# epruesse/SINA

Hardware: AMD Instinct MI355X
Metric: aligned sequences/sec (whole node), 100k full-length 16S vs SILVA-NR-scale ref (higher is better)
Workload: dtype f32

## Files before the change

sina_amd/csrc/graph_build.hip:

```cpp
#include <algorithm>
#include <cstring>
#include <type_traits>

#include "common.h"
#include "ctx.h"

namespace sina_hip {
namespace {

#ifndef SINA_GRAPH_THREADS
#define SINA_GRAPH_THREADS 512
#endif
#ifndef SINA_GRAPH_MINWAVES
#define SINA_GRAPH_MINWAVES 8
#endif
constexpr int kGT = SINA_GRAPH_THREADS;
constexpr uint32_t kNoPrev = 0xFFFFu;
constexpr int kMaxFam = kFamilyMax;
#ifndef SINA_GRAPH_KTC
#define SINA_GRAPH_KTC 128
#endif
#ifndef SINA_GRAPH_TNW
#define SINA_GRAPH_TNW 512
#endif
constexpr int kTC = SINA_GRAPH_KTC;
constexpr int kTNW = SINA_GRAPH_TNW;
static_assert(kTC % 64 == 0 && kTC < 255 && kTNW >= 32 && kTNW % 2 == 0, "tile geometry");
static_assert((kMaxFam * (kTC / 64) + SINA_GRAPH_THREADS / 64 - 1) / (SINA_GRAPH_THREADS / 64) <= 64, "far-entry flags of a wave fit 64 bits");

#ifdef SINA_DP_PROFILE
__device__ unsigned long long g_graph_prof[16];
#define GP_DECL unsigned long long gp_[16] = {}; unsigned long long gt_ = __builtin_amdgcn_s_memtime();
#define GP(i) { const unsigned long long t_ = __builtin_amdgcn_s_memtime(); gp_[i] += t_ - gt_; gt_ = t_; }
#define GP_FLUSH if (threadIdx.x == 0) { for (int i_ = 0; i_ < 16; i_++) atomicAdd(&g_graph_prof[i_], gp_[i_]); }
#else
#define GP_DECL
#define GP(i)
#define GP_FLUSH
#endif

struct GraphArgs {
    const uint32_t *ref_ab;
    const uint64_t *ref_off;
    const uint32_t *fam_ids;
    const uint64_t *fam_off;
    const uint64_t *pred_off;
    const float *wtab;
    uint4 *rec;
    uint32_t *node_pos;
    uint32_t *succ_min;
    uint32_t *far_mark;
    uint32_t *pred;
    uint2 *pred4;
    uint32_t *sizes;
    uint16_t *chain_rows;
    uint32_t width, ncap;
    uint32_t tile_bytes;
    uint32_t bitmap_off;
    uint32_t member_off;
    uint32_t member_cap;
    uint32_t fam_cap;
    int W;
    int want_smin;
    uint2 *reach;
    float kappa64;
};

struct Member {
    uint64_t beg;
    uint32_t len;
    uint32_t cur, curn;
    uint32_t carry, carryn;
    uint32_t id;
};
static_assert(sizeof(Member) == 32, "LDS layout");
constexpr uint32_t kOCpos = 0;
constexpr uint32_t kONbase = kOCpos + 4 * kTC;
constexpr uint32_t kOPres = kONbase + 4 * (kTC + 2);
constexpr uint32_t kOWA = kOPres + 4 * kTC;
constexpr uint32_t kOWC = kOWA + 4 * kTNW;
constexpr uint32_t kOWD = kOWC + 4 * kTNW;
constexpr uint32_t kOWB = (kOWD + 4 * kTNW + 7) & ~7u;
constexpr uint32_t kOLi = kOWB + 8 * kTNW;
constexpr uint32_t kONn = kOLi + 32 * kTC;
constexpr uint32_t kONfar = kONn + kTC;
constexpr uint32_t kOMask = kONfar + kTNW;
constexpr uint32_t kONcol = kOMask + kTNW;
constexpr uint32_t kOE = (kONcol + kTNW + 15) & ~15u;
constexpr int kELower0Bit = 14;
constexpr uint32_t kODot16 = kTC + 1;

template <typename In, typename Out>
__device__ uint32_t block_exscan(const In *in, Out *out, uint32_t n, uint32_t *tmp) {
    const uint32_t tid = threadIdx.x;
    const uint32_t chunk = (n + kGT - 1) / kGT;
    const uint32_t b = min(n, tid * chunk), e = min(n, b + chunk);
    uint32_t s = 0;
    for (uint32_t i = b; i < e; i++) s += (uint32_t)in[i];
    uint32_t x = s;
    const int lane = tid & 63, wave = tid >> 6;
#pragma unroll
    for (int off = 1; off < 64; off <<= 1) {
        const uint32_t y = __shfl_up(x, off);
        if (lane >= off) x += y;
    }
    if (lane == 63) tmp[wave] = x;
    __syncthreads();
    uint32_t base = 0, total = 0;
    for (int w = 0; w < kGT / 64; w++) {
        if (w < wave) base += tmp[w];
        total += tmp[w];
    }
    uint32_t run = base + x - s;
    __syncthreads();
    for (uint32_t i = b; i < e; i++) {
        const uint32_t v = (uint32_t)in[i];
        out[i] = (Out)run;
        run += v;
    }
    __syncthreads();
    return total;
}

template <typename Get, typename Out>
__device__ uint32_t block_exscan_f(uint32_t n, Get get, Out *out, uint32_t *tmp) {
    const uint32_t tid = threadIdx.x;
    const uint32_t chunk = (n + kGT - 1) / kGT;
    const uint32_t b = min(n, tid * chunk), e = min(n, b + chunk);
    uint32_t s = 0;
    for (uint32_t i = b; i < e; i++) s += get(i);
    uint32_t x = s;
    const int lane = tid & 63, wave = tid >> 6;
#pragma unroll
    for (int off = 1; off < 64; off <<= 1) {
        const uint32_t y = __shfl_up(x, off);
        if (lane >= off) x += y;
    }
    if (lane == 63) tmp[wave] = x;
    __syncthreads();
    uint32_t base = 0, total = 0;
    for (int w = 0; w < kGT / 64; w++) {
        if (w < wave) base += tmp[w];
        total += tmp[w];
    }
    uint32_t run = base + x - s;
    __syncthreads();
    for (uint32_t i = b; i < e; i++) {
        const uint32_t v = get(i);
        out[i] = (Out)run;
        run += v;
    }
    __syncthreads();
    return total;
}

__device__ __attribute__((noinline)) void fill_tile(const uint32_t *__restrict__ ref_ab, uint32_t bitmap_off, uint32_t member_off,
                                                    uint32_t nwords, uint32_t n_tasks, uint32_t c0, uint32_t tc) {
    extern __shared__ __attribute__((aligned(16))) unsigned char smem[];
    uint32_t *cposT = reinterpret_cast<uint32_t *>(smem + kOCpos);
    uint32_t *presT = reinterpret_cast<uint32_t *>(smem + kOPres);
    uint16_t *eE = reinterpret_cast<uint16_t *>(smem + kOE);
    const uint32_t *bitmap = reinterpret_cast<const uint32_t *>(smem + bitmap_off);
    const uint16_t *wrank = reinterpret_cast<const uint16_t *>(bitmap + nwords);
    Member *mb = reinterpret_cast<Member *>(smem + member_off);
    constexpr uint32_t kEAbsent = 0x00FFu, kEFirst = 1u << 13;
    constexpr uint32_t kCH = kTC / 64, kNW = kGT / 64;
    const uint32_t wave = (uint32_t)__builtin_amdgcn_readfirstlane((int)(threadIdx.x >> 6));
    const uint32_t lane = threadIdx.x & 63u;
    auto rank = [&](uint32_t pos) -> uint32_t {
        return (uint32_t)wrank[pos >> 5] + __popc(bitmap[pos >> 5] & ((1u << (pos & 31)) - 1u));
    };
        for (uint32_t t4 = wave; t4 < n_tasks; t4 += 8 * kNW) {
            uint32_t abv[8];
#pragma unroll
            for (int u = 0; u < 8; u++) {
                const uint32_t task = t4 + (uint32_t)u * kNW;
                abv[u] = 0xFFFFFFFFu;
                if (task < n_tasks) {
                    const uint32_t j = task / kCH;
                    const uint32_t cur = (uint32_t)__builtin_amdgcn_readfirstlane((int)mb[j].cur);
                    const uint32_t len = (uint32_t)__builtin_amdgcn_readfirstlane((int)mb[j].len);
                    const uint64_t beg = mb[j].beg;
                    const uint64_t begs = ((uint64_t)(uint32_t)__builtin_amdgcn_readfirstlane((int)(uint32_t)(beg >> 32)) << 32) |
                                          (uint32_t)__builtin_amdgcn_readfirstlane((int)(uint32_t)beg);
                    const uint32_t i = cur + (task % kCH) * 64u + lane;
                    if (i < len) abv[u] = ref_ab[begs + i];
                }
            }
#pragma unroll
            for (int u = 0; u < 8; u++) {
                const uint32_t task = t4 + (uint32_t)u * kNW;
                if (task >= n_tasks) continue;
                const uint32_t j = task / kCH, slot0 = (task % kCH) * 64u, slot = slot0 + lane;
                const uint32_t cur = (uint32_t)__builtin_amdgcn_readfirstlane((int)mb[j].cur);
                uint32_t ev = kEAbsent;
                if (abv[u] != 0xFFFFFFFFu) {
                    const uint32_t ab = abv[u];
                    const uint32_t pos = ab & 0xFFFFFFu;
                    const uint32_t c = rank(pos) - c0;
                    if (c < tc) {
                        const uint32_t m = (ab >> 24) & 0x1Fu;
                        ev = c | (m << 8) | (cur + slot == 0 ? kEFirst : 0u);
                        atomicOr(&presT[c], 1u << m);
                        cposT[c] = pos;
                    }
                }
                eE[j * (uint32_t)kTC + slot] = (uint16_t)ev;
                const uint32_t n_in = (uint32_t)__popcll(__builtin_amdgcn_ballot_w64(ev != kEAbsent));
                if (n_in && lane == 0) atomicMax(&mb[j].curn, cur + slot0 + n_in);
            }
        }
}

__device__ __forceinline__ uint32_t node_of_entry(uint32_t ev) {
    extern __shared__ __attribute__((aligned(16))) unsigned char smem[];
    const uint32_t *nbaseT = reinterpret_cast<const uint32_t *>(smem + kONbase);
    const uint32_t *presT = reinterpret_cast<const uint32_t *>(smem + kOPres);
    const uint8_t *liOf = smem + kOLi;
    const uint32_t c = ev & 0xFFu, m = (ev >> 8) & 31u;
    const uint32_t b = nbaseT[c];
    return b + liOf[b + __popc(presT[c] & ((1u << m) - 1u))];
}
__device__ __attribute__((noinline)) void merge_dot16(uint32_t n_tasks) {
    extern __shared__ __attribute__((aligned(16))) unsigned char smem[];
    const uint32_t *presT = reinterpret_cast<const uint32_t *>(smem + kOPres);
    uint16_t *eE = reinterpret_cast<uint16_t *>(smem + kOE);
    for (uint32_t e = threadIdx.x; e < n_tasks * 64u; e += kGT) {
        const uint32_t ev = eE[e];
        const uint32_t c = ev & 0xFFu;
        if (c != 0xFFu && ((ev >> 8) & 31u) == 16u && !(presT[c] & 0x10000u)) eE[e] = (uint16_t)((ev & ~(31u << 8)) | (1u << kELower0Bit));
    }
}
__device__ __attribute__((noinline)) void fix_dot16(uint32_t n_tasks, uint32_t ca, uint32_t cb, uint32_t w0) {
    extern __shared__ __attribute__((aligned(16))) unsigned char smem[];
    const uint32_t *nbaseT = reinterpret_cast<const uint32_t *>(smem + kONbase);
    const uint32_t *wC = reinterpret_cast<const uint32_t *>(smem + kOWC);
    const uint16_t *eE = reinterpret_cast<const uint16_t *>(smem + kOE);
    uint8_t *maskN = smem + kOMask;
    for (uint32_t e = threadIdx.x; e < n_tasks * 64u; e += kGT) {
        const uint32_t ev = eE[e];
        const uint32_t c = ev & 0xFFu;
        if (c >= ca && c < cb && (ev >> kELower0Bit) && wC[nbaseT[c] - w0] == e / (uint32_t)kTC) maskN[node_of_entry(ev) - w0] = 16;
    }
}
__global__ void __launch_bounds__(kGT) __attribute__((amdgpu_waves_per_eu(SINA_GRAPH_MINWAVES, SINA_GRAPH_MINWAVES))) family_graph_kernel(GraphArgs a) {
    extern __shared__ __attribute__((aligned(16))) unsigned char smem[];
    __shared__ uint32_t s_tmp[kGT / 64 + 8];
    const uint32_t q = blockIdx.x, tid = threadIdx.x;
    const uint32_t nwords = (a.width + 31) / 32;
    const uint64_t f0 = a.fam_off[q];
    const uint32_t F = (uint32_t)(a.fam_off[q + 1] - f0);
    uint32_t *cposT = reinterpret_cast<uint32_t *>(smem + kOCpos);
    uint32_t *nbaseT = reinterpret_cast<uint32_t *>(smem + kONbase);
    uint32_t *presT = reinterpret_cast<uint32_t *>(smem + kOPres);
    uint32_t *wA = reinterpret_cast<uint32_t *>(smem + kOWA);
    uint32_t *wC = reinterpret_cast<uint32_t *>(smem + kOWC);
    uint32_t *wD = reinterpret_cast<uint32_t *>(smem + kOWD);
    unsigned long long *wB = reinterpret_cast<unsigned long long *>(smem + kOWB);
    uint8_t *liOf = smem + kOLi;
    uint8_t *nn = smem + kONn;
    uint8_t *nfarN = smem + kONfar;
    uint8_t *maskN = smem + kOMask;
    uint8_t *ncolN = smem + kONcol;
    uint16_t *eE = reinterpret_cast<uint16_t *>(smem + kOE);
    uint32_t *bitmap = reinterpret_cast<uint32_t *>(smem + a.bitmap_off);
    uint16_t *wrank = reinterpret_cast<uint16_t *>(bitmap + nwords);
    Member *mb = reinterpret_cast<Member *>(smem + a.member_off);
    constexpr uint32_t kEFirst = 1u << 13;
    constexpr uint32_t kCH = kTC / 64, kNW = kGT / 64;
    const uint32_t wave = (uint32_t)__builtin_amdgcn_readfirstlane((int)(threadIdx.x >> 6));
    const uint32_t lane = threadIdx.x & 63u;
    const uint32_t n_tasks = F * kCH;

    uint32_t *sz = a.sizes + kBuiltWords * (size_t)q;
    for (uint32_t j = tid; j < F; j += kGT) {
        const uint32_t id = a.fam_ids[f0 + j];
        mb[j].id = id;
        mb[j].beg = a.ref_off[id];
        mb[j].len = (uint32_t)(a.ref_off[id + 1] - a.ref_off[id]);
        mb[j].cur = mb[j].curn = 0;
        mb[j].carry = mb[j].carryn = kNoPrev;
    }
    for (uint32_t i = tid; i < nwords; i += kGT) bitmap[i] = 0;
    if (tid == 0) nbaseT[kODot16] = 0;
    __syncthreads();
    GP_DECL

    for (uint32_t j0 = 0; j0 < F; j0 += 8) {
        uint32_t maxlen = 0;
#pragma unroll
        for (int u = 0; u < 8; u++) maxlen = max(maxlen, j0 + u < F ? mb[j0 + u].len : 0u);
        for (uint32_t i = tid; i < maxlen; i += kGT) {
            uint32_t ab[8];
#pragma unroll
            for (int u = 0; u < 8; u++)
                ab[u] = (j0 + u < F && i < mb[j0 + u].len) ? a.ref_ab[mb[j0 + u].beg + i] : 0xFFFFFFFFu;
#pragma unroll
            for (int u = 0; u < 8; u++)
                if (ab[u] != 0xFFFFFFFFu) {
                    const uint32_t pos = ab[u] & 0xFFFFFFu;
                    atomicOr(&bitmap[pos >> 5], 1u << (pos & 31));
                }
        }
    }
    __syncthreads();
    GP(0)
    {
        const uint32_t chunk = (nwords + kGT - 1) / kGT;
        const uint32_t b = min(nwords, tid * chunk), e = min(nwords, b + chunk);
        uint32_t s = 0;
        for (uint32_t i = b; i < e; i++) s += __popc(bitmap[i]);
        uint32_t x = s;
        const int lane = tid & 63, wave = tid >> 6;
#pragma unroll
        for (int off = 1; off < 64; off <<= 1) {
            const uint32_t y = __shfl_up(x, off);
            if (lane >= off) x += y;
        }
        if (lane == 63) s_tmp[wave] = x;
        __syncthreads();
        uint32_t base = 0, total = 0;
        for (int w = 0; w < kGT / 64; w++) {
            if (w < wave) base += s_tmp[w];
            total += s_tmp[w];
        }
        uint32_t run = base + x - s;
        for (uint32_t i = b; i < e; i++) {
            wrank[i] = (uint16_t)run;
            run += __popc(bitmap[i]);
        }
        if (tid == 0) s_tmp[kGT / 64] = total;
    }
    __syncthreads();
    const uint32_t NC = s_tmp[kGT / 64];
    if (NC > 65535u) {
        if (tid == 0) {
            sz[kBuiltN] = NC;
            sz[kBuiltEdges] = sz[kBuiltSpill] = 0;
            sz[kBuiltStatus] = kBuiltNodeCap;
        }
        return;
    }
    auto rank = [&](uint32_t pos) -> uint32_t {
        return (uint32_t)wrank[pos >> 5] + __popc(bitmap[pos >> 5] & ((1u << (pos & 31)) - 1u));
    };
    uint4 *rec = a.rec + (size_t)q * a.ncap;
    uint32_t *node_pos = a.node_pos + (size_t)q * a.ncap;
    uint32_t *smin = a.succ_min + (size_t)q * a.ncap;
    uint32_t *last = a.far_mark + (size_t)q * a.ncap;
    uint32_t *pred = a.pred + a.pred_off[q];
    uint16_t *chain_rows = a.chain_rows + (size_t)q * a.ncap;
    const float *wt = a.wtab + (size_t)F * (kMaxFam + 1);
    uint32_t N = 0, E = 0;
    GP(1)

    for (uint32_t c0 = 0; c0 < NC; c0 += kTC) {
        const uint32_t tc = min((uint32_t)kTC, NC - c0);
        for (uint32_t i = tid; i < (uint32_t)kTC; i += kGT) presT[i] = 0;
        __syncthreads();
        GP(2)
        fill_tile(a.ref_ab, a.bitmap_off, a.member_off, nwords, n_tasks, c0, tc);
        __syncthreads();
        for (uint32_t c = tid; c < tc; c += kGT) {
            uint32_t p = presT[c];
            if ((p & 0x10001u) == 0x10001u) {
                p &= ~0x10000u;
                presT[c] = p;
                nbaseT[kODot16] = 1u;
            }
            nn[c] = (uint8_t)__popc(p);
        }
        __syncthreads();
        if (nbaseT[kODot16]) {
            merge_dot16(n_tasks);
            __syncthreads();
        }
        GP(3)
        const uint32_t tn = block_exscan(nn, nbaseT, tc, s_tmp);
        if (tid == 0) nbaseT[tc] = tn;
        for (uint32_t ln = tid; ln < tn; ln += kGT)
            if (N + ln < a.ncap) {
                last[N + ln] = 0;
                if (a.want_smin) smin[N + ln] = 0xFFFFFFFFu;
            }
        __syncthreads();
        GP(5)
        uint32_t te = 0;
        for (uint32_t ca = 0; ca < tc;) {
            const uint32_t w0 = nbaseT[ca];
            uint32_t cb = tc;
            if (tn - w0 > (uint32_t)kTNW) {
                uint32_t lo = ca + 1, hi = tc;
                while (lo < hi) {
                    const uint32_t mid = (lo + hi + 1) / 2;
                    if (nbaseT[mid] - w0 <= (uint32_t)kTNW) lo = mid;
                    else hi = mid - 1;
                }
                cb = lo;
            }
            const uint32_t wn = nbaseT[cb] - w0;
            for (uint32_t i = tid; i < wn; i += kGT) {
                wA[i] = 0;
                wB[i] = 0;
                wC[i] = 0xFFFFFFFFu;
                nfarN[i] = 0;
            }
            __syncthreads();
            for (uint32_t task = wave; task < n_tasks; task += kNW) {
                const uint32_t j = task / kCH, slot = (task % kCH) * 64u + lane;
                const uint32_t ev = eE[j * (uint32_t)kTC + slot];
                const uint32_t c = ev & 0xFFu;
                if (c >= ca && c < cb) {
                    const uint32_t m = (ev >> 8) & 31u;
                    atomicMin(&wC[nbaseT[c] + __popc(presT[c] & ((1u << m) - 1u)) - w0], j);
                }
            }
            __syncthreads();
            for (uint32_t c = ca + tid; c < cb; c += kGT) {
                const uint32_t base = nbaseT[c], k = nn[c];
                uint32_t pp = presT[c];
                for (uint32_t x = 0; x < k; x++) {
                    const uint32_t mj = wC[base - w0 + x];
                    uint32_t r = 0;
                    for (uint32_t y = 0; y < k; y++) r += (wC[base - w0 + y] < mj) ? 1u : 0u;
                    liOf[base + x] = (uint8_t)r;
                    maskN[base - w0 + r] = (uint8_t)(__ffs(pp) - 1);
                    ncolN[base - w0 + r] = (uint8_t)c;
                    pp &= pp - 1u;
                }
            }
            __syncthreads();
            if (nbaseT[kODot16]) {
                fix_dot16(n_tasks, ca, cb, w0);
                __syncthreads();
            }
            GP(4)
            auto node_of = [&](uint32_t ev) -> uint32_t { return node_of_entry(ev); };
            unsigned long long farbits = 0;
            {
                uint32_t it = 0;
                for (uint32_t task = wave; task < n_tasks; task += kNW, it++) {
                    const uint32_t j = task / kCH, slot = (task % kCH) * 64u + lane;
                    const uint32_t ev = eE[j * (uint32_t)kTC + slot];
                    const uint32_t c = ev & 0xFFu;
                    const bool mine = c >= ca && c < cb;
                    const uint32_t ln = mine ? node_of(ev) : 0u;
                    uint32_t lnp = __shfl_up(ln, 1);
                    const bool left_mine = __shfl_up(mine ? 1 : 0, 1) != 0;
                    if (!mine) continue;
                    const uint32_t node = N + ln;
                    const bool first = (ev & kEFirst) != 0;
                    atomicAdd(&wA[ln - w0], first ? 1u : 0x10001u);
                    if (mb[j].cur + slot + 1 == mb[j].curn) mb[j].carryn = node;
                    if (j == 0 && mb[0].cur + slot < a.ncap) chain_rows[mb[0].cur + slot] = (uint16_t)node;
                    if (!first) {
                        if (slot && (lane == 0 || !left_mine)) lnp = node_of(eE[j * (uint32_t)kTC + slot - 1]);
                        const uint32_t pn = slot ? N + lnp : mb[j].carry;
                        const uint32_t d = node - pn;
                        if (d <= 64u) atomicOr(&wB[ln - w0], 1ull << (d - 1u));
                        else farbits |= 1ull << it;
                    }
                }
            }
            for (uint32_t i = tid; i < wn; i += kGT) wC[i] = 0xFFFFFFFFu;
            __syncthreads();
            GP(6)
            const uint32_t te_w = block_exscan_f(wn, [&](uint32_t i) { return wA[i] >> 16; }, wD, s_tmp);
            while (__syncthreads_or(farbits != 0 ? 1 : 0)) {
                uint32_t it = 0;
                for (uint32_t task = wave; task < n_tasks; task += kNW, it++) {
                    if (!((farbits >> it) & 1ull)) continue;
                    const uint32_t j = task / kCH, slot = (task % kCH) * 64u + lane;
                    const uint32_t ln = node_of(eE[j * (uint32_t)kTC + slot]);
                    const uint32_t pn = slot ? N + node_of(eE[j * (uint32_t)kTC + slot - 1]) : mb[j].carry;
                    atomicMin(&wC[ln - w0], pn);
                }
                __syncthreads();
                it = 0;
                for (uint32_t task = wave; task < n_tasks; task += kNW, it++) {
                    if (!((farbits >> it) & 1ull)) continue;
                    const uint32_t j = task / kCH, slot = (task % kCH) * 64u + lane;
                    const uint32_t ln = node_of(eE[j * (uint32_t)kTC + slot]);
                    const uint32_t pn = slot ? N + node_of(eE[j * (uint32_t)kTC + slot - 1]) : mb[j].carry;
                    if (wC[ln - w0] == pn) farbits &= ~(1ull << it);
                }
                __syncthreads();
                for (uint32_t i = tid; i < wn; i += kGT) {
                    const uint32_t v = wC[i];
                    if (v == 0xFFFFFFFFu) continue;
                    const uint32_t node = N + w0 + i;
                    if (node < a.ncap) {
                        pred[E + te + wD[i] + nfarN[i]] = v;
                        if (a.want_smin) atomicMin(&smin[v], cposT[ncolN[i]]);
                        atomicMax(&last[v], node);
                    }
                    nfarN[i]++;
                    wC[i] = 0xFFFFFFFFu;
                }
            }
            for (uint32_t i = tid; i < wn; i += kGT) {
                const uint32_t node = N + w0 + i;
                if (node >= a.ncap) continue;
                const uint32_t seg = E + te + wD[i];
                const uint32_t pos = cposT[ncolN[i]];
                uint32_t np = nfarN[i];
                unsigned long long bits = wB[i];
                while (bits) {
                    const uint32_t hi = 63u - (uint32_t)__clzll((long long)bits);
                    bits ^= 1ull << hi;
                    const uint32_t pa = node - (hi + 1u);
                    pred[seg + np] = pa;
                    np++;
                    if (a.want_smin) atomicMin(&smin[pa], pos);
                    atomicMax(&last[pa], node);
                }
                uint4 r;
                r.x = seg;
                r.y = __float_as_uint(wt[wA[i] & 0xFFFFu]);
                r.z = (np & 0xFFu) | ((uint32_t)maskN[i] << 8);
                r.w = kRowNone;
                rec[node] = r;
                node_pos[node] = pos;
            }
            te += te_w;
            ca = cb;
            __syncthreads();
        }
        for (uint32_t j = tid; j < F; j += kGT) {
            mb[j].cur = mb[j].curn;
            mb[j].carry = mb[j].carryn;
        }
        N += tn;
        E += te;
        __syncthreads();
        GP(7)
    }
    if (N > a.ncap || N > 65535u) {
        if (tid == 0) {
            sz[kBuiltN] = N;
            sz[kBuiltEdges] = sz[kBuiltSpill] = 0;
            sz[kBuiltStatus] = kBuiltNodeCap;
        }
        return;
    }
    GP(8)
    const uint32_t seg_len = dp_slot_segment(N);
    const uint32_t n_seg = (N + seg_len - 1) / seg_len;
    uint32_t *codeL = reinterpret_cast<uint32_t *>(smem);
    const bool in_lds = (size_t)N * 4 <= a.tile_bytes;
    if (tid == 0) s_tmp[kGT / 64 + 1] = 0xFFFFFFFFu;
    __syncthreads();
    for (uint32_t i = tid; i < N; i += kGT) {
        uint32_t z = rec[i].z;
        const uint32_t l = last[i];
        if (l == 0) {
            z |= kRecSink;
            atomicMin(&s_tmp[kGT / 64 + 1], i);
            if (a.want_smin) smin[i] = 1000000u;
        }
        if (l > i && l - i > (uint32_t)kFarLds) z |= kRecFence;
        rec[i].z = z;
        if (in_lds) codeL[i] = l | ((z & kRecSink) ? (1u << 30) : 0u) | ((z & kRecFence) ? (1u << 31) : 0u);
    }
    __syncthreads();
    GP(9)
    if (tid < n_seg) {
        auto walk = [&](auto kslots) {
            constexpr int K = decltype(kslots)::value;
            uint32_t fa[K];
#pragma unroll
            for (int x = 0; x < K; x++) fa[x] = (x < a.W) ? 0u : 0xFFFFFFFFu;
            uint32_t nsp = 0;
            const uint32_t b = tid * seg_len, e = min(N, b + seg_len);
            for (uint32_t m = b; m < e; m++) {
                uint32_t l, sink, fence;
                if (in_lds) {
                    const uint32_t cd = codeL[m];
                    l = cd & 0xFFFFu;
                    sink = cd & (1u << 30);
                    fence = cd & (1u << 31);
                } else {
                    const uint32_t z = rec[m].z;
                    l = last[m];
                    sink = z & kRecSink;
                    fence = z & kRecFence;
                }
                uint32_t wv = kRowNone;
                if (!sink && l != m + 1) {
                    const bool may_slot = !fence && l < e;
                    uint32_t slot = K;
#pragma unroll
                    for (int x = K - 1; x >= 0; x--) slot = (may_slot && fa[x] <= m) ? (uint32_t)x : slot;
#pragma unroll
                    for (int x = 0; x < K; x++) fa[x] = (slot == (uint32_t)x) ? l : fa[x];
                    wv = slot < (uint32_t)K ? slot : (kRowSpilled | nsp++);
                }
                if (in_lds) codeL[m] = wv;
                else rec[m].w = wv;
            }
            mb[tid].id = nsp;
        };
        if (a.W <= 4) walk(std::integral_constant<int, 4>());
        else walk(std::integral_constant<int, 8>());
    }
    __syncthreads();
    {
        uint32_t tot = 0;
        for (uint32_t g = 0; g < n_seg; g++) tot += mb[g].id;
        for (uint32_t i = tid; i < N; i += kGT) {
            uint32_t w = in_lds ? codeL[i] : rec[i].w;
            if (w != kRowNone && (w & kRowSpilled)) {
                uint32_t base = 0;
                for (uint32_t g = 0; g < i / seg_len; g++) base += mb[g].id;
                w += base;
            }
            rec[i].w = w;
            if (in_lds) codeL[i] = w;
        }
        if (tid == 0) {
            sz[kBuiltN] = N;
            sz[kBuiltEdges] = E;
            sz[kBuiltSpill] = tot;
            sz[kBuiltStatus] = (tot > kMaxSpillRows) ? kBuiltSpillCap : 0u;
            sz[kBuiltFirstSink] = s_tmp[kGT / 64 + 1];
            sz[kBuiltChainLen] = mb[0].len;
        }
    }
    __syncthreads();
    GP(10)
    uint2 *pred4 = a.pred4 + (size_t)q * a.ncap;
    for (uint32_t i = tid; i < N; i += kGT) {
        const uint4 r = rec[i];
        const uint32_t np = r.z & 0xFFu;
        uint32_t first_far = 0;
        uint32_t dist = np ? 0u : kRecDistFar;
        uint32_t p4[4] = {0u, 0u, 0u, 0u};
        for (uint32_t x = 0; x < np; x++) {
            const uint32_t pa = pred[r.x + x];
            uint32_t pw = in_lds ? codeL[pa] : rec[pa].w;
            if (pw == kRowNone) pw = 0;
            const bool sp = (pw & kRowSpilled) != 0;
            if (sp && first_far == 0) first_far = x + 1;
            dist = max(dist, i - pa);
            pred[r.x + x] = pa | ((pw & 0x7FFFu) << 16) | (sp ? kPredSpilled : 0u);
            if (x == 0) p4[0] = pa;
            else if (x == 1) p4[1] = pa;
            else if (x == 2) p4[2] = pa;
            else if (x == 3) p4[3] = pa;
        }
        rec[i].z = r.z | (first_far << 24) | (min(dist, kRecDistFar) << kRecDistShift);
        pred4[i] = pred4_pack(p4[0], p4[1], p4[2], p4[3]);
    }
    GP(11)
    if (a.reach != nullptr) {
        uint2 *rg = a.reach + (size_t)q * a.ncap;
        uint32_t *cw = in_lds ? codeL : (a.want_smin ? last : smin);
        if (tid == 0) s_tmp[kGT / 64 + 2] = 0xFFFFFFFFu;
        __syncthreads();
        for (uint32_t i = tid; i < N; i += kGT) {
            const uint32_t pos = node_pos[i];
            if (i > 0 && node_pos[i - 1] == pos) continue;
            uint32_t mx = 0;
            for (uint32_t j = i; j < N && node_pos[j] == pos; j++) {
                mx = max(mx, prune_gain_units(__uint_as_float(rec[j].y), a.kappa64));
                cw[j] = 0;
            }
            cw[i] = mx;
            atomicMin(&s_tmp[kGT / 64 + 2], mx);
        }
        __syncthreads();
        if (tid == 0) sz[kBuiltGmin] = s_tmp[kGT / 64 + 2];
        const uint32_t total = block_exscan(cw, cw, N, s_tmp);
        for (uint32_t i = tid; i < N; i += kGT) {
            const uint32_t pos = node_pos[i];
            if (i > 0 && node_pos[i - 1] == pos) continue;
            const uint32_t right = (i + 1 < N) ? total - cw[i + 1] : 0u;
            const uint32_t cols_right = NC - 1u - rank(pos);
            for (uint32_t j = i; j < N && node_pos[j] == pos; j++) rg[j] = uint2{right, ((a.want_smin && !in_lds) ? 0u : last[j]) | (cols_right << 16)};
        }
    }
    GP(12)
    GP_FLUSH
}

size_t graph_bitmap_off(uint32_t max_family) { return ((size_t)kOE + 2 * (size_t)max_family * kTC + 15) & ~(size_t)15; }
size_t graph_lds_bytes(uint32_t width, uint32_t max_family) {
    const size_t nwords = (width + 31) / 32;
    return graph_bitmap_off(max_family) + ((6 * nwords + 15) & ~(size_t)15);
}
size_t graph_member_cap(uint32_t max_family) { return std::max<size_t>(16, (max_family + 1) & ~(size_t)1); }
size_t graph_lds_total(uint32_t width, uint32_t max_family) {
    return graph_lds_bytes(width, max_family) + sizeof(Member) * graph_member_cap(max_family);
}

}
}

using namespace sina_hip;

namespace {

int build_family_graphs(sina_hip_ctx *c, const uint32_t *fam_ids, const uint64_t *fam_off, uint32_t q0,
                        uint32_t bq, float fs_weight, int W, BuiltGraphs *bg, bool want_smin, float kappa64, bool for_dp) {
    hipStream_t s = c->stream;
    if (ensure_ref_off_host(c)) return 1;
    std::vector<uint64_t> foff(bq + 1), elems(bq, 0);
    uint32_t max_f = 1;
    bg->pred_off.assign(bq, 0);
    for (uint32_t q = 0; q <= bq; q++) foff[q] = fam_off[q0 + q] - fam_off[q0];
    for (uint32_t q = 0; q < bq; q++) {
        max_f = std::max<uint32_t>(max_f, (uint32_t)(foff[q + 1] - foff[q]));
        for (uint64_t x = fam_off[q0 + q]; x < fam_off[q0 + q + 1]; x++) {
            const uint32_t id = fam_ids[x];
            if (id >= c->st->n_refs) SH_FAIL("align_families: reference id out of range");
            elems[q] += c->st->ref_off_host[id + 1] - c->st->ref_off_host[id];
        }
        if (for_dp && elems[q] == 0) SH_FAIL("align_families: a family without a single base");
    }
    if (!(c->wtab_fs_weight == fs_weight) || !c->g_wtab.p) {
        std::vector<float> wt((size_t)(kMaxFam + 1) * (kMaxFam + 1), 0.f);
        const float weight = fs_weight;
        for (unsigned F = 1; F <= (unsigned)kMaxFam; F++)
            for (unsigned cnt = 0; cnt <= F; cnt++)
                wt[(size_t)F * (kMaxFam + 1) + cnt] =
                    (float)(1.0 / (double)(weight + 1) + (double)(weight * ((float)cnt / (float)F)));
        if (c->g_wtab.reserve(wt.size() * 4)) return 1;
        SH_CHECK(hipMemcpyAsync(c->g_wtab.p, wt.data(), wt.size() * 4, hipMemcpyHostToDevice, s));
        SH_CHECK(hipStreamSynchronize(s));
        c->wtab_fs_weight = fs_weight;
    }
    uint32_t ncap = std::min<uint32_t>(65535, 12288);
    for (int attempt = 0;; attempt++) {
        uint64_t pred_total = 0;
        for (uint32_t q = 0; q < bq; q++) {
            bg->pred_off[q] = pred_total;
            pred_total += elems[q] + 8;
        }
        const size_t glds_tables = graph_lds_bytes(c->st->width, max_f);
        const size_t glds = graph_lds_total(c->st->width, max_f);
        if (glds > 160 * 1024) SH_FAIL_LIMIT("align_families: family too wide for the device DAG build");
        if (c->g_fam_ids.reserve(4 * std::max<uint64_t>(foff[bq], 1)) || c->g_fam_off.reserve(8 * ((uint64_t)bq + 1)) ||
            c->g_tmp1.reserve(8 * (uint64_t)bq) ||
            c->rec.reserve(sizeof(uint4) * (uint64_t)bq * ncap) || c->node_pos.reserve(4 * (uint64_t)bq * ncap) ||
            c->succ_minpos.reserve(4 * (uint64_t)bq * ncap) || c->g_tmp3.reserve(4 * (uint64_t)bq * ncap) ||
            c->pred.reserve(4 * pred_total) || c->pred4.reserve(sizeof(uint2) * (uint64_t)bq * ncap) || c->g_sizes.reserve(4 * kBuiltWords * (uint64_t)bq) ||
            c->scout.reserve(2 * (uint64_t)bq * ncap) ||
            (kappa64 > 0.f && c->rgain.reserve(8 * (uint64_t)bq * ncap)))
            return 1;
        if (upload(c, 1, c->g_fam_ids.p, fam_ids + fam_off[q0], 4 * foff[bq], s) ||
            upload(c, 2, c->g_fam_off.p, foff.data(), 8 * ((uint64_t)bq + 1), s) ||
            upload(c, 3, c->g_tmp1.p, bg->pred_off.data(), 8 * (uint64_t)bq, s))
            return 1;
        GraphArgs ga;
        ga.ref_ab = c->st->ref_ab.as<uint32_t>();
        ga.ref_off = c->st->ref_off.as<uint64_t>();
        ga.fam_ids = c->g_fam_ids.as<uint32_t>();
        ga.fam_off = c->g_fam_off.as<uint64_t>();
        ga.pred_off = c->g_tmp1.as<uint64_t>();
        ga.wtab = c->g_wtab.as<float>();
        ga.rec = c->rec.as<uint4>();
        ga.node_pos = c->node_pos.as<uint32_t>();
        ga.succ_min = c->succ_minpos.as<uint32_t>();
        ga.far_mark = c->g_tmp3.as<uint32_t>();
        ga.pred = c->pred.as<uint32_t>();
        ga.pred4 = c->pred4.as<uint2>();
        ga.sizes = c->g_sizes.as<uint32_t>();
        ga.chain_rows = c->scout.as<uint16_t>();
        ga.width = c->st->width;
        ga.ncap = ncap;
        ga.bitmap_off = (uint32_t)graph_bitmap_off(max_f);
        ga.tile_bytes = ga.bitmap_off;
        ga.member_off = (uint32_t)glds_tables;
        ga.member_cap = (uint32_t)graph_member_cap(max_f);
        ga.fam_cap = max_f;
        ga.W = W;
        ga.want_smin = want_smin ? 1 : 0;
        ga.reach = kappa64 > 0.f ? c->rgain.as<uint2>() : nullptr;
        ga.kappa64 = kappa64;
        if (allow_full_lds(reinterpret_cast<const void *>(family_graph_kernel))) return 1;
        bg->sizes.resize(kBuiltWords * (size_t)bq);
        {
            heavy_launch hl(c, s, kHeavyGraph);
            SH_CHECK(hipEventRecord(c->ev[6], hl.stream()));
            hipLaunchKernelGGL(family_graph_kernel, dim3(bq), dim3(kGT), glds, hl.stream(), ga);
            SH_CHECK(hipGetLastError());
            SH_CHECK(hipEventRecord(c->ev[7], hl.stream()));
            if (hl.done()) return 1;
        }
        if (download(c, 4, c->g_sizes.p, 4 * kBuiltWords * (uint64_t)bq, s)) return 1;
        SH_CHECK(wait_stream(c, s));
        memcpy(bg->sizes.data(), c->h_stage[4].p, 4 * kBuiltWords * (uint64_t)bq);
        float gms = 0;
        SH_CHECK(hipEventElapsedTime(&gms, c->ev[6], c->ev[7]));
        {
            uint64_t bytes = 0;
            for (uint32_t q = 0; q < bq; q++)
                bytes += 4 * elems[q] + (uint64_t)bg->sizes[kBuiltWords * q + kBuiltN] * (16 + 4 + 8 + (kappa64 > 0.f ? 8 : 0)) +
                         4 * (uint64_t)bg->sizes[kBuiltWords * q + kBuiltEdges];
            std::lock_guard<std::mutex> slk(c->st->stats_mu);
            c->st->stats.graph_ms += gms;
            c->st->stats.graph_bytes += bytes;
            c->st->stats.graph_launches++;
        }
        uint32_t need_n = 0;
        for (uint32_t q = 0; q < bq; q++) {
            const uint32_t status = bg->sizes[kBuiltWords * q + kBuiltStatus];
            if (status == kBuiltNodeCap) need_n = std::max(need_n, bg->sizes[kBuiltWords * q + kBuiltN]);
            if (status == kBuiltSpillCap) SH_FAIL_LIMIT("align_families: too many spill rows for one query");
        }
        if (!need_n) break;
        if (attempt >= 3 || need_n > 65535u) SH_FAIL_LIMIT("align_families: family DAG exceeds device limits");
        ncap = std::min<uint32_t>(65535, need_n + need_n / 8 + 16);
    }
    bg->ncap = ncap;
    return 0;
}

int build_graphs_for_launch(sina_hip_ctx *c, const uint32_t *fam_ids, const uint64_t *fam_off, uint32_t q0, uint32_t n,
                            const sina_hip_align_params *p, int W, const PrunePlan &pp, BuiltGraphs *bg) {
    return build_family_graphs(c, fam_ids, fam_off, q0, n, p->fs_weight, W, bg, p->insertion == SINA_INSERTION_FORBID,
                               pp.on ? pp.kappa64 : 0.f, true);
}

}

extern "C" {

int sina_hip_align_families(sina_hip_ctx *c, const uint32_t *fam_ids, const uint64_t *fam_off, uint32_t nq,
                            const uint8_t *qmask, const uint64_t *qoff, const sina_hip_align_params *p,
                            sina_hip_align_out *out, uint32_t *out_pos) {
    return align_family_batches(c, FamilyCall{"align_families", build_graphs_for_launch, false, fam_ids, fam_off, nq, qmask, qoff, p, out, out_pos});
}

int sina_hip_align_families_wsets(sina_hip_ctx *c, const uint32_t *fam_ids, const uint64_t *fam_off, uint32_t nq,
                                  const uint8_t *qmask, const uint64_t *qoff, const sina_hip_align_params *p,
                                  const uint32_t *weight_set, uint32_t n_sets, sina_hip_align_out *out, uint32_t *out_pos) {
    if (p && !weighted_scheme(p)) SH_FAIL("align_families_wsets: weight sets need positional weights (p->weights, p->n_weights)");
    return align_family_batches(c, FamilyCall{"align_families_wsets", build_graphs_for_launch, false, fam_ids, fam_off, nq, qmask, qoff, p,
                                             out, out_pos, weight_set, n_sets});
}

#ifdef SINA_DP_PROFILE
int sina_hip_debug_graph_profile(unsigned long long *out16, int reset) {
    SH_CHECK(hipMemcpyFromSymbol(out16, HIP_SYMBOL(g_graph_prof), sizeof(unsigned long long) * 16));
    if (reset) {
        unsigned long long z[16] = {};
        SH_CHECK(hipMemcpyToSymbol(HIP_SYMBOL(g_graph_prof), z, sizeof z));
    }
    return 0;
}
#endif

int sina_hip_debug_family_graph(sina_hip_ctx *c, const uint32_t *fam_ids, uint32_t F, float fs_weight,
                                uint32_t ring_depth, uint32_t *n_nodes, uint32_t *n_edges, uint32_t *pos,
                                uint8_t *mask, float *weight, uint32_t *pred_off, uint32_t *pred,
                                uint32_t *succ_minpos, uint8_t *sink, uint32_t *spill_idx, uint32_t cap_nodes,
                                uint32_t cap_edges) {
    if (!c || !fam_ids || !n_nodes || !n_edges) SH_FAIL("debug_family_graph: null argument");
    std::lock_guard<std::mutex> lk(c->mu);
    if (!c->st->have_refs) SH_FAIL("debug_family_graph: upload references first");
    if (F == 0 || F > (uint32_t)kMaxFam) SH_FAIL("debug_family_graph: family size must be in 1..128");
    SH_CHECK(hipSetDevice(c->device));
    const uint64_t foff[2] = {0, F};
    BuiltGraphs bg;
    if (build_family_graphs(c, fam_ids, foff, 0, 1, fs_weight, (int)ring_depth, &bg, true, fs_weight >= 0.f ? 64.0f * 1.0001f * 2.0f : 0.f, false)) return 1;
    const uint32_t N = bg.sizes[kBuiltN];
    std::vector<uint4> rec(N);
    std::vector<uint32_t> pr(bg.sizes[kBuiltEdges] + 8);
    SH_CHECK(hipMemcpy(rec.data(), c->rec.p, sizeof(uint4) * N, hipMemcpyDeviceToHost));
    SH_CHECK(hipMemcpy(pr.data(), c->pred.p, 4 * pr.size(), hipMemcpyDeviceToHost));
    uint32_t E = 0;
    for (uint32_t m = 0; m < N; m++) E += rec[m].z & 0xffu;
    *n_nodes = N;
    *n_edges = E;
    if (N > cap_nodes || E > cap_edges) SH_FAIL("debug_family_graph: output buffers too small");
    SH_CHECK(hipMemcpy(pos, c->node_pos.p, 4 * N, hipMemcpyDeviceToHost));
    SH_CHECK(hipMemcpy(succ_minpos, c->succ_minpos.p, 4 * N, hipMemcpyDeviceToHost));
    uint32_t e = 0;
    for (uint32_t m = 0; m < N; m++) {
        mask[m] = (uint8_t)((rec[m].z >> 8) & 0xffu);
        memcpy(&weight[m], &rec[m].y, 4);
        sink[m] = (rec[m].z & kRecSink) ? 1 : 0;
        spill_idx[m] = rec[m].w;
        pred_off[m] = e;
        for (uint32_t x = 0; x < (rec[m].z & 0xffu); x++) pred[e++] = pr[rec[m].x + x] & 0xffffu;
    }
    pred_off[N] = e;
    return 0;
}

int sina_hip_debug_family_graph_words(sina_hip_ctx *c, const uint32_t *fam_ids, uint32_t F, float fs_weight,
                                      uint32_t ring_depth, uint32_t *n_nodes, uint32_t *n_edges, uint32_t *rec_z,
                                      uint32_t *rec_w, uint32_t *pred_entries, uint32_t *size_words, uint32_t cap_nodes,
                                      uint32_t cap_edges) {
    if (!c || !fam_ids || !n_nodes || !n_edges || !rec_z || !rec_w || !pred_entries || !size_words)
        SH_FAIL("debug_family_graph_words: null argument");
    std::lock_guard<std::mutex> lk(c->mu);
    if (!c->st->have_refs) SH_FAIL("debug_family_graph_words: upload references first");
    if (F == 0 || F > (uint32_t)kMaxFam) SH_FAIL("debug_family_graph_words: family size must be in 1..128");
    SH_CHECK(hipSetDevice(c->device));
    const uint64_t foff[2] = {0, F};
    BuiltGraphs bg;
    if (build_family_graphs(c, fam_ids, foff, 0, 1, fs_weight, (int)ring_depth, &bg, true, fs_weight >= 0.f ? 64.0f * 1.0001f * 2.0f : 0.f, false)) return 1;
    const uint32_t N = bg.sizes[kBuiltN];
    std::vector<uint4> rec(N);
    std::vector<uint32_t> pr(bg.sizes[kBuiltEdges] + 8);
    if (N) SH_CHECK(hipMemcpy(rec.data(), c->rec.p, sizeof(uint4) * N, hipMemcpyDeviceToHost));
    SH_CHECK(hipMemcpy(pr.data(), c->pred.p, 4 * pr.size(), hipMemcpyDeviceToHost));
    uint32_t E = 0;
    for (uint32_t m = 0; m < N; m++) E += rec[m].z & 0xffu;
    *n_nodes = N;
    *n_edges = E;
    if (N > cap_nodes || E > cap_edges) SH_FAIL("debug_family_graph_words: output buffers too small");
    uint32_t e = 0;
    for (uint32_t m = 0; m < N; m++) {
        rec_z[m] = rec[m].z;
        rec_w[m] = rec[m].w;
        for (uint32_t x = 0; x < (rec[m].z & 0xffu); x++) pred_entries[e++] = pr[rec[m].x + x];
    }
    memcpy(size_words, bg.sizes.data(), 4 * kBuiltWords);
    return 0;
}

}
```

Before: 300,100.

## Overlap slot walk with column-maxima scan and fuse rec/pred finalization passes

After: 305,600, median of 6. +1.8%, better.

```diff
diff --git a/sina_amd/csrc/graph_build.hip b/sina_amd/csrc/graph_build.hip
--- a/sina_amd/csrc/graph_build.hip
+++ b/sina_amd/csrc/graph_build.hip
@@ -152,6 +152,64 @@
     }
     __syncthreads();
     return total;
+}
+
+__device__ uint32_t block_incscan(uint32_t *v, uint32_t n, uint32_t *tmp) {
+    const uint32_t tid = threadIdx.x;
+    const uint32_t chunk = (n + kGT - 1) / kGT;
+    const uint32_t b = min(n, tid * chunk), e = min(n, b + chunk);
+    uint32_t s = 0;
+    for (uint32_t i = b; i < e; i++) s += v[i];
+    uint32_t x = s;
+    const int lane = tid & 63, wave = tid >> 6;
+#pragma unroll
+    for (int off = 1; off < 64; off <<= 1) {
+        const uint32_t y = __shfl_up(x, off);
+        if (lane >= off) x += y;
+    }
+    if (lane == 63) tmp[wave] = x;
+    __syncthreads();
+    uint32_t base = 0, total = 0;
+    for (int w = 0; w < kGT / 64; w++) {
+        if (w < wave) base += tmp[w];
+        total += tmp[w];
+    }
+    uint32_t run = base + x - s;
+    for (uint32_t i = b; i < e; i++) {
+        run += v[i];
+        v[i] = run;
+    }
+    __syncthreads();
+    return total;
+}
+
+constexpr uint32_t kCdSpilled = 1u << 16, kCdNone = 1u << 17, kCdSink = 1u << 30, kCdFence = 1u << 31;
+__device__ __forceinline__ uint32_t row_of_code(uint32_t c) {
+    return (c & kCdNone) ? kRowNone : (c & kCdSpilled) ? (kRowSpilled | (c & 0xFFFFu)) : (c & 0xFFFFu);
+}
+
+template <int K, typename Get, typename Put>
+__device__ __forceinline__ uint32_t slot_walk(uint32_t b, uint32_t e, int W, Get get, Put put) {
+    uint32_t fa[K];
+#pragma unroll
+    for (int x = 0; x < K; x++) fa[x] = (x < W) ? 0u : 0xFFFFFFFFu;
+    uint32_t nsp = 0;
+    for (uint32_t m = b; m < e; m++) {
+        const uint32_t cd = get(m);
+        const uint32_t l = cd & 0xFFFFu;
+        uint32_t c = kCdNone;
+        if (!(cd & kCdSink) && l != m + 1) {
+            const bool may_slot = !(cd & kCdFence) && l < e;
+            uint32_t slot = K;
+#pragma unroll
+            for (int x = K - 1; x >= 0; x--) slot = (may_slot && fa[x] <= m) ? (uint32_t)x : slot;
+#pragma unroll
+            for (int x = 0; x < K; x++) fa[x] = (slot == (uint32_t)x) ? l : fa[x];
+            c = slot < (uint32_t)K ? slot : (kCdSpilled | nsp++);
+        }
+        put(m, cd, c);
+    }
+    return nsp;
 }
 
 __device__ __attribute__((noinline)) void fill_tile(const uint32_t *__restrict__ ref_ab, uint32_t bitmap_off, uint32_t member_off,
@@ -548,116 +606,28 @@
     const uint32_t n_seg = (N + seg_len - 1) / seg_len;
     uint32_t *codeL = reinterpret_cast<uint32_t *>(smem);
     const bool in_lds = (size_t)N * 4 <= a.tile_bytes;
-    if (tid == 0) s_tmp[kGT / 64 + 1] = 0xFFFFFFFFu;
+    const bool beside = a.reach != nullptr && (size_t)N * 8 <= a.tile_bytes;
+    uint32_t *cwL = codeL + N;
+    constexpr int kSFirstSink = kGT / 64 + 1, kSGmin = kGT / 64 + 2, kSSpill = kGT / 64 + 3;
+    if (tid == 0) {
+        s_tmp[kSFirstSink] = 0xFFFFFFFFu;
+        s_tmp[kSGmin] = 0xFFFFFFFFu;
+    }
     __syncthreads();
     for (uint32_t i = tid; i < N; i += kGT) {
-        uint32_t z = rec[i].z;
         const uint32_t l = last[i];
+        uint32_t cd = l;
         if (l == 0) {
-            z |= kRecSink;
-            atomicMin(&s_tmp[kGT / 64 + 1], i);
+            cd |= kCdSink;
+            atomicMin(&s_tmp[kSFirstSink], i);
             if (a.want_smin) smin[i] = 1000000u;
         }
-        if (l > i && l - i > (uint32_t)kFarLds) z |= kRecFence;
-        rec[i].z = z;
-        if (in_lds) codeL[i] = l | ((z & kRecSink) ? (1u << 30) : 0u) | ((z & kRecFence) ? (1u << 31) : 0u);
-    }
-    __syncthreads();
-    GP(9)
-    if (tid < n_seg) {
-        auto walk = [&](auto kslots) {
-            constexpr int K = decltype(kslots)::value;
-            uint32_t fa[K];
-#pragma unroll
-            for (int x = 0; x < K; x++) fa[x] = (x < a.W) ? 0u : 0xFFFFFFFFu;
-            uint32_t nsp = 0;
-            const uint32_t b = tid * seg_len, e = min(N, b + seg_len);
-            for (uint32_t m = b; m < e; m++) {
-                uint32_t l, sink, fence;
-                if (in_lds) {
-                    const uint32_t cd = codeL[m];
-                    l = cd & 0xFFFFu;
-                    sink = cd & (1u << 30);
-                    fence = cd & (1u << 31);
-                } else {
-                    const uint32_t z = rec[m].z;
-                    l = last[m];
-                    sink = z & kRecSink;
-                    fence = z & kRecFence;
-                }
-                uint32_t wv = kRowNone;
-                if (!sink && l != m + 1) {
-                    const bool may_slot = !fence && l < e;
-                    uint32_t slot = K;
-#pragma unroll
-                    for (int x = K - 1; x >= 0; x--) slot = (may_slot && fa[x] <= m) ? (uint32_t)x : slot;
-#pragma unroll
-                    for (int x = 0; x < K; x++) fa[x] = (slot == (uint32_t)x) ? l : fa[x];
-                    wv = slot < (uint32_t)K ? slot : (kRowSpilled | nsp++);
-                }
-                if (in_lds) codeL[m] = wv;
-                else rec[m].w = wv;
-            }
-            mb[tid].id = nsp;
-        };
-        if (a.W <= 4) walk(std::integral_constant<int, 4>());
-        else walk(std::integral_constant<int, 8>());
-    }
-    __syncthreads();
-    {
-        uint32_t tot = 0;
-        for (uint32_t g = 0; g < n_seg; g++) tot += mb[g].id;
-        for (uint32_t i = tid; i < N; i += kGT) {
-            uint32_t w = in_lds ? codeL[i] : rec[i].w;
-            if (w != kRowNone && (w & kRowSpilled)) {
-                uint32_t base = 0;
-                for (uint32_t g = 0; g < i / seg_len; g++) base += mb[g].id;
-                w += base;
-            }
-            rec[i].w = w;
-            if (in_lds) codeL[i] = w;
-        }
-        if (tid == 0) {
-            sz[kBuiltN] = N;
-            sz[kBuiltEdges] = E;
-            sz[kBuiltSpill] = tot;
-            sz[kBuiltStatus] = (tot > kMaxSpillRows) ? kBuiltSpillCap : 0u;
-            sz[kBuiltFirstSink] = s_tmp[kGT / 64 + 1];
-            sz[kBuiltChainLen] = mb[0].len;
-        }
-    }
-    __syncthreads();
-    GP(10)
-    uint2 *pred4 = a.pred4 + (size_t)q * a.ncap;
-    for (uint32_t i = tid; i < N; i += kGT) {
-        const uint4 r = rec[i];
-        const uint32_t np = r.z & 0xFFu;
-        uint32_t first_far = 0;
-        uint32_t dist = np ? 0u : kRecDistFar;
-        uint32_t p4[4] = {0u, 0u, 0u, 0u};
-        for (uint32_t x = 0; x < np; x++) {
-            const uint32_t pa = pred[r.x + x];
-            uint32_t pw = in_lds ? codeL[pa] : rec[pa].w;
-            if (pw == kRowNone) pw = 0;
-            const bool sp = (pw & kRowSpilled) != 0;
-            if (sp && first_far == 0) first_far = x + 1;
-            dist = max(dist, i - pa);
-            pred[r.x + x] = pa | ((pw & 0x7FFFu) << 16) | (sp ? kPredSpilled : 0u);
-            if (x == 0) p4[0] = pa;
-            else if (x == 1) p4[1] = pa;
-            else if (x == 2) p4[2] = pa;
-            else if (x == 3) p4[3] = pa;
-        }
-        rec[i].z = r.z | (first_far << 24) | (min(dist, kRecDistFar) << kRecDistShift);
-        pred4[i] = pred4_pack(p4[0], p4[1], p4[2], p4[3]);
-    }
-    GP(11)
-    if (a.reach != nullptr) {
-        uint2 *rg = a.reach + (size_t)q * a.ncap;
-        uint32_t *cw = in_lds ? codeL : (a.want_smin ? last : smin);
-        if (tid == 0) s_tmp[kGT / 64 + 2] = 0xFFFFFFFFu;
-        __syncthreads();
-        for (uint32_t i = tid; i < N; i += kGT) {
+        if (l > i && l - i > (uint32_t)kFarLds) cd |= kCdFence;
+        if (in_lds) codeL[i] = cd;
+        else if (cd & (kCdSink | kCdFence)) rec[i].z |= ((cd & kCdSink) ? kRecSink : 0u) | ((cd & kCdFence) ? kRecFence : 0u);
+    }
+    auto column_maxima = [&](uint32_t *cw, uint32_t first, uint32_t step) {
+        for (uint32_t i = first; i < N; i += step) {
             const uint32_t pos = node_pos[i];
             if (i > 0 && node_pos[i - 1] == pos) continue;
             uint32_t mx = 0;
@@ -666,20 +636,148 @@
                 cw[j] = 0;
             }
             cw[i] = mx;
-            atomicMin(&s_tmp[kGT / 64 + 2], mx);
+            atomicMin(&s_tmp[kSGmin], mx);
+        }
+    };
+    __syncthreads();
+    GP(9)
+    if (wave == 0) {
+        uint32_t nsp = 0;
+        if (tid < n_seg) {
+            const uint32_t b = tid * seg_len, e = min(N, b + seg_len);
+            auto walk = [&](auto kslots) {
+                constexpr int K = decltype(kslots)::value;
+                if (in_lds)
+                    return slot_walk<K>(b, e, a.W, [&](uint32_t m) { return codeL[m]; },
+                                        [&](uint32_t m, uint32_t cd, uint32_t c) { codeL[m] = (cd & (kCdSink | kCdFence)) | c; });
+                return slot_walk<K>(b, e, a.W,
+                                    [&](uint32_t m) {
+                                        const uint32_t z = rec[m].z;
+                                        return last[m] | ((z & kRecSink) ? kCdSink : 0u) | ((z & kRecFence) ? kCdFence : 0u);
+                                    },
+                                    [&](uint32_t m, uint32_t, uint32_t c) { rec[m].w = row_of_code(c); });
+            };
+            nsp = (a.W <= 4) ? walk(std::integral_constant<int, 4>()) : walk(std::integral_constant<int, 8>());
+        }
+        uint32_t x = nsp;
+#pragma unroll
+        for (int off = 1; off < 16; off <<= 1) {
+            const uint32_t y = __shfl_up(x, off);
+            if (lane >= (uint32_t)off) x += y;
+        }
+        if (tid < n_seg) mb[tid].id = x - nsp;
+        if (tid == 15) s_tmp[kSSpill] = x;
+    } else if (beside) {
+        column_maxima(cwL, tid - 64u, (uint32_t)kGT - 64u);
+    }
+    __syncthreads();
+    const uint32_t tot = s_tmp[kSSpill];
+    if (tid == 0) {
+        sz[kBuiltN] = N;
+        sz[kBuiltEdges] = E;
+        sz[kBuiltSpill] = tot;
+        sz[kBuiltStatus] = (tot > kMaxSpillRows) ? kBuiltSpillCap : 0u;
+        sz[kBuiltFirstSink] = s_tmp[kSFirstSink];
+        sz[kBuiltChainLen] = mb[0].len;
+        if (beside) sz[kBuiltGmin] = s_tmp[kSGmin];
+    }
+    uint2 *pred4 = a.pred4 + (size_t)q * a.ncap;
+    uint2 *rg = a.reach + (size_t)q * a.ncap;
+    if (in_lds) {
+        for (uint32_t i = tid; i < N; i += kGT) {
+            const uint32_t c = codeL[i];
+            if (c & kCdSpilled) codeL[i] = c + mb[i / seg_len].id;
+        }
+        uint32_t total = 0;
+        if (beside) total = block_incscan(cwL, N, s_tmp);
+        else __syncthreads();
+        GP(10)
+        for (uint32_t i = tid; i < N; i += kGT) {
+            const uint4 r = rec[i];
+            const uint32_t cd = codeL[i];
+            const uint32_t np = r.z & 0xFFu;
+            uint32_t first_far = 0;
+            uint32_t dist = np ? 0u : kRecDistFar;
+            uint32_t p4[4] = {0u, 0u, 0u, 0u};
+            for (uint32_t x = 0; x < np; x++) {
+                const uint32_t pa = pred[r.x + x];
+                const uint32_t pc = codeL[pa];
+                const bool sp = (pc & kCdSpilled) != 0;
+                if (sp && first_far == 0) first_far = x + 1;
+                dist = max(dist, i - pa);
+                pred[r.x + x] = pa | ((pc & 0x7FFFu) << 16) | (sp ? kPredSpilled : 0u);
+                if (x == 0) p4[0] = pa;
+                else if (x == 1) p4[1] = pa;
+                else if (x == 2) p4[2] = pa;
+                else if (x == 3) p4[3] = pa;
+            }
+            uint4 o;
+            o.x = r.x;
+            o.y = r.y;
+            o.z = r.z | ((cd & kCdSink) ? kRecSink : 0u) | ((cd & kCdFence) ? kRecFence : 0u) | (first_far << 24) |
+                  (min(dist, kRecDistFar) << kRecDistShift);
+            o.w = row_of_code(cd);
+            rec[i] = o;
+            pred4[i] = pred4_pack(p4[0], p4[1], p4[2], p4[3]);
+            if (beside) rg[i] = uint2{total - cwL[i], last[i] | ((NC - 1u - rank(node_pos[i])) << 16)};
+        }
+        GP(11)
+        if (a.reach != nullptr && !beside) {
+            __syncthreads();
+            column_maxima(codeL, tid, (uint32_t)kGT);
+            __syncthreads();
+            if (tid == 0) sz[kBuiltGmin] = s_tmp[kSGmin];
+            total = block_incscan(codeL, N, s_tmp);
+            for (uint32_t i = tid; i < N; i += kGT)
+                rg[i] = uint2{total - codeL[i], last[i] | ((NC - 1u - rank(node_pos[i])) << 16)};
+        }
+        GP(12)
+    } else {
+        for (uint32_t i = tid; i < N; i += kGT) {
+            const uint32_t w = rec[i].w;
+            if (w != kRowNone && (w & kRowSpilled)) rec[i].w = w + mb[i / seg_len].id;
         }
         __syncthreads();
-        if (tid == 0) sz[kBuiltGmin] = s_tmp[kGT / 64 + 2];
-        const uint32_t total = block_exscan(cw, cw, N, s_tmp);
+        GP(10)
         for (uint32_t i = tid; i < N; i += kGT) {
-            const uint32_t pos = node_pos[i];
-            if (i > 0 && node_pos[i - 1] == pos) continue;
-            const uint32_t right = (i + 1 < N) ? total - cw[i + 1] : 0u;
-            const uint32_t cols_right = NC - 1u - rank(pos);
-            for (uint32_t j = i; j < N && node_pos[j] == pos; j++) rg[j] = uint2{right, ((a.want_smin && !in_lds) ? 0u : last[j]) | (cols_right << 16)};
-        }
-    }
-    GP(12)
+            const uint4 r = rec[i];
+            const uint32_t np = r.z & 0xFFu;
+            uint32_t first_far = 0;
+            uint32_t dist = np ? 0u : kRecDistFar;
+            uint32_t p4[4] = {0u, 0u, 0u, 0u};
+            for (uint32_t x = 0; x < np; x++) {
+                const uint32_t pa = pred[r.x + x];
+                uint32_t pw = rec[pa].w;
+                if (pw == kRowNone) pw = 0;
+                const bool sp = (pw & kRowSpilled) != 0;
+                if (sp && first_far == 0) first_far = x + 1;
+                dist = max(dist, i - pa);
+                pred[r.x + x] = pa | ((pw & 0x7FFFu) << 16) | (sp ? kPredSpilled : 0u);
+                if (x == 0) p4[0] = pa;
+                else if (x == 1) p4[1] = pa;
+                else if (x == 2) p4[2] = pa;
+                else if (x == 3) p4[3] = pa;
+            }
+            rec[i].z = r.z | (first_far << 24) | (min(dist, kRecDistFar) << kRecDistShift);
+            pred4[i] = pred4_pack(p4[0], p4[1], p4[2], p4[3]);
+        }
+        GP(11)
+        if (a.reach != nullptr) {
+            uint32_t *cw = a.want_smin ? last : smin;
+            column_maxima(cw, tid, (uint32_t)kGT);
+            __syncthreads();
+            if (tid == 0) sz[kBuiltGmin] = s_tmp[kSGmin];
+            const uint32_t total = block_exscan(cw, cw, N, s_tmp);
+            for (uint32_t i = tid; i < N; i += kGT) {
+                const uint32_t pos = node_pos[i];
+                if (i > 0 && node_pos[i - 1] == pos) continue;
+                const uint32_t right = (i + 1 < N) ? total - cw[i + 1] : 0u;
+                const uint32_t cols_right = NC - 1u - rank(pos);
+                for (uint32_t j = i; j < N && node_pos[j] == pos; j++) rg[j] = uint2{right, (a.want_smin ? 0u : last[j]) | (cols_right << 16)};
+            }
+        }
+        GP(12)
+    }
     GP_FLUSH
 }
 
```
